# nktoan/h-edit

Measured on AMD Instinct MI355X. Metric: edited images/sec (512^2, 50 steps, K Langevin), higher is better.
Workload: dtype bf16

## Files before the change

h-edit_amd/csrc/attn.hip:

```cpp
#include "common.h"
#include "kernels.h"
#include <type_traits>

namespace {

typedef __attribute__((ext_vector_type(4))) unsigned u32x4;

__device__ __forceinline__ float fast_exp2(float x) { return __builtin_amdgcn_exp2f(x); }
#ifndef SA_BURST
#define SA_BURST 0
#endif

template <int D>
struct HeadCfg {
  static constexpr int DP = (D + 15) / 16 * 16;
  static constexpr int DK = DP / 16;
  static constexpr int DT = (D + 31) / 32;
  static constexpr int KS = DP + 8;
  static constexpr int DCH = D / 8;
};

__device__ __forceinline__ bf16x8 pack_p8(const float* p) {
  union { uint32_t u[4]; bf16x8 v; } x;
  x.u[0] = pack_bf16x2(p[0], p[1]);
// ... 427 lines not shown
      block(integral_constant<int, 0>{}, false_type{}, false_type{}, U);
      block(integral_constant<int, 1>{}, false_type{}, false_type{}, U + 1);
      if (QG == 2) hand_over((U >> 2) + 1); else hand_over((U >> 1) + 2);
      block(integral_constant<int, 2>{}, false_type{}, false_type{}, U + 2);
      block(integral_constant<int, 3>{}, false_type{}, false_type{}, U + 3);
      U = 4;
    }
    for (; U + 6 <= TU; U += 4) {
      if (QG == 1) hand_over((U >> 1) + 1);
      block(integral_constant<int, 0>{}, false_type{}, pin, U);
      block(integral_constant<int, 1>{}, false_type{}, pin, U + 1);
      if (QG == 2) hand_over((U >> 2) + 1); else hand_over((U >> 1) + 2);
      block(integral_constant<int, 2>{}, false_type{}, pin, U + 2);
      block(integral_constant<int, 3>{}, false_type{}, pin, U + 3);
    }
    {
      if (QG == 1) hand_over((U >> 1) + 1);
      block(integral_constant<int, 0>{}, true_type{}, pin, U);
      block(integral_constant<int, 1>{}, true_type{}, pin, U + 1);
      if (U + 2 < TU) {
        if (QG == 2) hand_over((U >> 2) + 1); else hand_over((U >> 1) + 2);
        block(integral_constant<int, 2>{}, true_type{}, pin, U + 2);
        block(integral_constant<int, 3>{}, true_type{}, pin, U + 3);
      }
    }
    {
      bf16x8 (&pf_last)[2] = pfb;
      constexpr int AL = NS - 1;
      if constexpr (PV16) {
#pragma unroll
        for (int gq = 0; gq < 2; ++gq)
#pragma unroll
          for (int dt = 0; dt < DT16; ++dt)
            o16[AL][gq][dt] = MFMA_16x16x32_ST(vf16[dt], pf_last[gq], o16[AL][gq][dt], 0, 0, 0);
      } else {
#pragma unroll
      for (int dt = 0; dt < DT; ++dt) o[AL][dt] = MFMA_32x32x16_ST(vf[dt][0], pf_last[0], o[AL][dt], 0, 0, 0);
#pragma unroll
      for (int dt = 0; dt < DT; ++dt) o[AL][dt] = MFMA_32x32x16_ST(vf[dt][1], pf_last[1], o[AL][dt], 0, 0, 0);
      }
    }
  };

  constexpr int dl = D - (DT - 1) * 32;
  constexpr int r1 = (dl & 3) + 4 * (dl >> 3);
  constexpr int h1 = (dl >> 2) & 1;
  auto denom16 = [&](int a, int gq) __attribute__((always_inline)) {
    return __shfl(o16[a][gq][D / 16][D % 4], 16 * ((D % 16) / 4) + (lane & 15), 64);
  };
  auto denom = [&](int a) __attribute__((always_inline)) {
    if (ONES) return __shfl(o[a][DT - 1][ONES ? r1 : 0], ql + 32 * h1, 64);
    return l_run[a] + __shfl_xor(l_run[a], 32, 64);
  };
  auto write_out = [&](const f32x16 (&acc)[DT], float inv, int q_row) __attribute__((always_inline)) {
    if (q_row < p.N) {
      bf16_t* op = p.out + ((long)b * p.N + q_row) * p.ldo + h * D;
#pragma unroll
      for (int dt = 0; dt < DT; ++dt)
#pragma unroll
        for (int gg = 0; gg < 4; ++gg) {
          const int d0 = dt * 32 + 8 * gg + 4 * hi;
          if (d0 < D) {
            uint2 w;
            w.x = pack_bf16x2(acc[dt][gg * 4 + 0] * inv, acc[dt][gg * 4 + 1] * inv);
            w.y = pack_bf16x2(acc[dt][gg * 4 + 2] * inv, acc[dt][gg * 4 + 3] * inv);
            *reinterpret_cast<uint2*>(op + d0) = w;
          }
        }
    }
  };
  {
    constexpr bool CAN_PIN = D != 64;
    int redo = 1;
    if (CAN_PIN && TU >= 6 && !(p.test_flags & 2)) {
      pass(true_type{});
      bool bad = false;
#pragma unroll
      for (int a = 0; a < NS; ++a) {
        constexpr float DEN_MAX = HEDIT_F16 ? 0x1p15f : 0x1p60f;
        if constexpr (PV16) bad |= !(denom16(a, 0) < DEN_MAX) || !(denom16(a, 1) < DEN_MAX);
        else bad |= !(denom(a) < DEN_MAX);
      }
      redo = __syncthreads_or(bad ? 1 : 0);
    }
    if (redo) pass(false_type{});
  }
  if constexpr (PV16) {
#pragma unroll
    for (int g = 0; g < 2; ++g)
#pragma unroll
      for (int gq = 0; gq < 2; ++gq) {
        const float inv = 1.0f / denom16(g, gq);
        const int q_row = qblk * (128 * QG) + wave * (32 * QG) + g * 32 + gq * 16 + (lane & 15);
        if (q_row < p.N) {
          bf16_t* op = p.out + ((long)b * p.N + q_row) * p.ldo + h * D;
#pragma unroll
          for (int dt = 0; dt < DT16; ++dt) {
            const int d0 = dt * 16 + 4 * (lane >> 4);
            if (d0 < D) {
              uint2 w;
              w.x = pack_bf16x2(o16[g][gq][dt][0] * inv, o16[g][gq][dt][1] * inv);
              w.y = pack_bf16x2(o16[g][gq][dt][2] * inv, o16[g][gq][dt][3] * inv);
              *reinterpret_cast<uint2*>(op + d0) = w;
            }
          }
        }
      }
  } else if (QG == 2) {
#pragma unroll
    for (int g = 0; g < 2; ++g) write_out(o[g], 1.0f / denom(g), q_base + g * 32);
  } else {
    if (NS == 2) {
      const float m = fmaxf(m_run[0], m_run[NS - 1]);
      const float f0 = fast_exp2(m_run[0] - m), f1 = fast_exp2(m_run[NS - 1] - m);
      if (!ONES) l_run[0] = l_run[0] * f0 + l_run[NS - 1] * f1;
#pragma unroll
      for (int dt = 0; dt < DT; ++dt)
#pragma unroll
        for (int r = 0; r < 16; ++r) o[0][dt][r] = o[0][dt][r] * f0 + o[NS - 1][dt][r] * f1;
    }
    write_out(o[0], 1.0f / denom(0), q_base);
  }
}

template <int D, int QG, int NS>
int launch_self(const SelfAttnParams& p, hipStream_t st) {
  using C = SelfCfg<D, QG>;
#ifdef SA_OCC1
  constexpr int LDS = C::TOTAL > 84 * 1024 ? C::TOTAL : 84 * 1024;
#else
  constexpr int LDS = C::TOTAL;
#endif
  if (int rc = hedit_dyn_lds(reinterpret_cast<const void*>(&self_attn_kernel<D, QG, NS>), LDS)) return rc;
  dim3 grid(cdiv(p.N, 128 * QG) * p.heads * p.B);
  hipLaunchKernelGGL((self_attn_kernel<D, QG, NS>), grid, dim3(256), LDS, st, p);
  LAUNCH_CHECK();
  return HEDIT_OK;
}

constexpr int CTXP = HEDIT_CTXP;
constexpr int WS = 100;

template <int D>
struct CrossSmem {
  using H = HeadCfg<D>;
  static constexpr int K_BYTES = 96 * H::KS * 2;
  static constexpr int V_BYTES = H::DT * 32 * WS * 2;
  static constexpr int MIX_BYTES = 96 * WS * 2;
  static constexpr int BV_BYTES = 96 * 4;
  static constexpr int TOTAL = K_BYTES + V_BYTES + MIX_BYTES + BV_BYTES;
};

template <int D>
__global__ __launch_bounds__(256, (D <= 80 ? 2 : 1)) void cross_attn_kernel(CrossAttnParams p) {
  using H = HeadCfg<D>;
  using S = CrossSmem<D>;
  extern __shared__ __attribute__((aligned(16))) char smem[];
  bf16_t* sK = reinterpret_cast<bf16_t*>(smem);
  bf16_t* sV = reinterpret_cast<bf16_t*>(smem + S::K_BYTES);
  bf16_t* sM = reinterpret_cast<bf16_t*>(smem + S::K_BYTES + S::V_BYTES);
  float* sB = reinterpret_cast<float*>(smem + S::K_BYTES + S::V_BYTES + S::MIX_BYTES);

  const int tid = threadIdx.x, lane = tid & 63, wave = tid >> 6;
  const int ql = lane & 31, hi = lane >> 5;
  const int h = blockIdx.y;
  const int item = blockIdx.z;
  const bool is_pair = item < p.n_pairs;
  const int b0 = is_pair ? p.pair_src[item] : p.singles[item - p.n_pairs];
  const int b1 = is_pair ? p.pair_tar[item] : -1;
  const int q_row = blockIdx.x * 128 + wave * 32 + ql;
  const bool q_ok = q_row < p.N;

  for (int i = tid; i < (S::K_BYTES + S::V_BYTES) / 8; i += 256) reinterpret_cast<uint2*>(smem)[i] = make_uint2(0, 0);
  if (is_pair) {
    const bf16_t* src = p.mixT + (long)item * 96 * 96;
    for (int i = tid; i < 96 * 12; i += 256) {
      const int row = i / 12, c = i - row * 12;
      const uint4 u = *reinterpret_cast<const uint4*>(src + row * 96 + c * 8);
      uint2* dst = reinterpret_cast<uint2*>(sM + row * WS + c * 8);
      dst[0] = make_uint2(u.x, u.y);
      dst[1] = make_uint2(u.z, u.w);
    }
    if (tid < 96) sB[tid] = p.bvec[(long)item * 96 + tid];
  }
  __syncthreads();

  auto stage = [&](int b) {
    const bf16_t* kbase = p.k + (long)b * CTXP * p.ldk + h * D;
    for (int idx = tid; idx < CTXP * H::DCH; idx += 256) {
      const int row = idx / H::DCH, c = idx - row * H::DCH;
      *reinterpret_cast<uint4*>(sK + row * H::KS + c * 8) =
          *reinterpret_cast<const uint4*>(kbase + (long)row * p.ldk + c * 8);
    }
    const bf16_t* vbase = p.vt + (long)h * D * p.ldvt + (long)b * CTXP;
    for (int idx = tid; idx < D * (CTXP / 8); idx += 256) {
      const int row = idx / (CTXP / 8), c = idx - row * (CTXP / 8);
      const uint4 u = *reinterpret_cast<const uint4*>(vbase + (long)row * p.ldvt + c * 8);
      uint2* dst = reinterpret_cast<uint2*>(sV + row * WS + c * 8);
      dst[0] = make_uint2(u.x, u.y);
      dst[1] = make_uint2(u.z, u.w);
    }
  };

  auto load_q = [&](int b, bf16x8* qf) {
    const bf16_t* qp = p.q + ((long)b * p.N + (q_ok ? q_row : 0)) * p.ldq + h * D;
#pragma unroll
    for (int ks = 0; ks < H::DK; ++ks) {
      const int c = ks * 16 + hi * 8;
      union { uint4 u; bf16x8 v; } x;
      x.u = make_uint4(0, 0, 0, 0);
      if (q_ok && c < D) x.u = *reinterpret_cast<const uint4*>(qp + c);
      qf[ks] = x.v;
    }
  };

  auto probs = [&](const bf16x8* qf, float (*pr)[16]) {
    float mx = -1e30f;
#pragma unroll
    for (int nt = 0; nt < 3; ++nt) {
      f32x16 s;
#pragma unroll
      for (int r = 0; r < 16; ++r) s[r] = 0.f;
#pragma unroll
      for (int ks = 0; ks < H::DK; ++ks) {
        const bf16x8 kf = *reinterpret_cast<const bf16x8*>(sK + (nt * 32 + ql) * H::KS + ks * 16 + hi * 8);
        s = MFMA_32x32x16_ST(kf, qf[ks], s, 0, 0, 0);
      }
#pragma unroll
      for (int r = 0; r < 16; ++r) {
        const int n = nt * 32 + (r & 3) + 8 * (r >> 2) + 4 * hi;
        const float v = n < HEDIT_MAXW ? s[r] : -1e30f;
        pr[nt][r] = v;
        mx = fmaxf(mx, v);
      }
    }
    mx = fmaxf(mx, __shfl_xor(mx, 32, 64));
    float ls = 0.f;
#pragma unroll
    for (int nt = 0; nt < 3; ++nt)
#pragma unroll
      for (int r = 0; r < 16; ++r) { pr[nt][r] = fast_exp2(pr[nt][r] - mx); ls += pr[nt][r]; }
    ls += __shfl_xor(ls, 32, 64);
    const float inv = 1.0f / ls;
#pragma unroll
    for (int nt = 0; nt < 3; ++nt)
#pragma unroll
      for (int r = 0; r < 16; ++r) pr[nt][r] *= inv;
  };

  auto accumulate_store = [&](int which, float (*pr)[16]) {
    if (p.store == nullptr || !q_ok) return;
    float* dst = p.store + ((((long)item * 2 + which) * p.heads + h) * p.N + q_row) * HEDIT_MAXW;
#pragma unroll
    for (int nt = 0; nt < 3; ++nt)
#pragma unroll
      for (int r = 0; r < 16; ++r) {
        const int n = nt * 32 + (r & 3) + 8 * (r >> 2) + 4 * hi;
        if (n < HEDIT_MAXW) dst[n] += pr[nt][r];
      }
  };

  auto pv_and_write = [&](int b, const bf16x8 (*pf)[2]) {
    f32x16 o[H::DT];
#pragma unroll
    for (int dt = 0; dt < H::DT; ++dt) {
#pragma unroll
      for (int r = 0; r < 16; ++r) o[dt][r] = 0.f;
#pragma unroll
      for (int nt = 0; nt < 3; ++nt)
#pragma unroll
        for (int s2 = 0; s2 < 2; ++s2) {
          const bf16x8 vf = read_perm_frag(sV, dt * 32 + ql, WS, nt * 32 + 16 * s2 + 4 * hi);
          o[dt] = MFMA_32x32x16_ST(vf, pf[nt][s2], o[dt], 0, 0, 0);
        }
    }
    if (q_ok) {
      bf16_t* op = p.out + ((long)b * p.N + q_row) * p.ldo + h * D;
#pragma unroll
      for (int dt = 0; dt < H::DT; ++dt)
#pragma unroll
        for (int g = 0; g < 4; ++g) {
          const int d0 = dt * 32 + 8 * g + 4 * hi;
          if (d0 < D) {
            uint2 w;
            w.x = pack_bf16x2(o[dt][g * 4 + 0], o[dt][g * 4 + 1]);
            w.y = pack_bf16x2(o[dt][g * 4 + 2], o[dt][g * 4 + 3]);
            *reinterpret_cast<uint2*>(op + d0) = w;
          }
        }
    }
  };

  bf16x8 qf[H::DK];
  float pr[3][16];
  bf16x8 pf[3][2];

  stage(b0);
  __syncthreads();
  load_q(b0, qf);
  probs(qf, pr);
  if (is_pair) accumulate_store(0, pr);
#pragma unroll
  for (int nt = 0; nt < 3; ++nt) { pf[nt][0] = pack_p8(pr[nt]); pf[nt][1] = pack_p8(pr[nt] + 8); }
  pv_and_write(b0, pf);
  if (!is_pair) return;

  f32x16 mix[3];
#pragma unroll
  for (int nt = 0; nt < 3; ++nt) {
#pragma unroll
    for (int r = 0; r < 16; ++r) mix[nt][r] = 0.f;
#pragma unroll
    for (int wt = 0; wt < 3; ++wt)
#pragma unroll
      for (int s2 = 0; s2 < 2; ++s2) {
        const bf16x8 mf = read_perm_frag(sM, nt * 32 + ql, WS, wt * 32 + 16 * s2 + 4 * hi);
        mix[nt] = MFMA_32x32x16_ST(mf, pf[wt][s2], mix[nt], 0, 0, 0);
      }
  }
  __syncthreads();
  stage(b1);
  __syncthreads();
  load_q(b1, qf);
  probs(qf, pr);
#pragma unroll
  for (int nt = 0; nt < 3; ++nt)
#pragma unroll
    for (int g = 0; g < 4; ++g) {
      const f32x4 bv = *reinterpret_cast<const f32x4*>(sB + nt * 32 + 8 * g + 4 * hi);
#pragma unroll
      for (int j = 0; j < 4; ++j) pr[nt][g * 4 + j] = mix[nt][g * 4 + j] + bv[j] * pr[nt][g * 4 + j];
    }
  accumulate_store(1, pr);
#pragma unroll
  for (int nt = 0; nt < 3; ++nt) { pf[nt][0] = pack_p8(pr[nt]); pf[nt][1] = pack_p8(pr[nt] + 8); }
  pv_and_write(b1, pf);
}

template <int D>
int launch_cross(const CrossAttnParams& p, hipStream_t st) {
  using S = CrossSmem<D>;
  if (int rc = hedit_dyn_lds(reinterpret_cast<const void*>(&cross_attn_kernel<D>), S::TOTAL)) return rc;
  dim3 grid(cdiv(p.N, 128), p.heads, p.n_pairs + p.n_single);
  hipLaunchKernelGGL((cross_attn_kernel<D>), grid, dim3(256), S::TOTAL, st, p);
  LAUNCH_CHECK();
  return HEDIT_OK;
}

template <bool STORE>
__global__ __launch_bounds__(256) void attn_probs_kernel(AttnProbsParams p) {
  __shared__ float qs[16][168];
  extern __shared__ float sc_rows[];
  const int bh = blockIdx.y, h = bh % p.heads;
  int b = bh / p.heads;
  if constexpr (STORE) {
    const int pair = b >> 1;
    b = (b & 1) ? p.pair_tar[pair] : p.pair_src[pair];
  }
  const int bq = (STORE && p.qk_src) ? p.qk_src[b] : b;
  const int q0 = blockIdx.x * 16, tid = threadIdx.x;
  for (int i = tid; i < 16 * p.d; i += 256) {
    const int r = i / p.d, c = i % p.d;
    const int q = q0 + r;
    qs[r][c] = q < p.N ? bf16_to_f32(p.q[((long)bq * p.N + q) * p.ldq + h * p.d + c]) : 0.f;
  }
  __syncthreads();
  float* out = STORE ? sc_rows : p.probs + ((long)bh * p.N + q0) * p.M;
  const int rows = min(16, p.N - q0);
  for (int m = tid; m < p.M; m += 256) {
    const bf16_t* kp = p.k + ((long)bq * p.kstride + m) * p.ldk + h * p.d;
    float acc[16];
#pragma unroll
    for (int r = 0; r < 16; ++r) acc[r] = 0.f;
    for (int c = 0; c < p.d; c += 8) {
      const uint4 raw = *reinterpret_cast<const uint4*>(kp + c);
      const uint32_t w[4] = {raw.x, raw.y, raw.z, raw.w};
#pragma unroll
      for (int j = 0; j < 8; ++j) {
        const float kv = (j & 1) ? st_hi(w[j >> 1]) : st_lo(w[j >> 1]);
#pragma unroll
        for (int r = 0; r < 16; ++r) acc[r] += qs[r][c + j] * kv;
      }
    }
    for (int r = 0; r < rows; ++r) out[(long)r * p.M + m] = acc[r];
  }
  __syncthreads();
  const int wave = tid >> 6, lane = tid & 63;
  for (int r = wave; r < rows; r += 4) {
    float* row = out + (long)r * p.M;
    float mx = -3.0e38f;
    for (int m = lane; m < p.M; m += 64) mx = fmaxf(mx, row[m]);
#pragma unroll
    for (int o = 32; o > 0; o >>= 1) mx = fmaxf(mx, __shfl_xor(mx, o, 64));
    float sum = 0.f;
    for (int m = lane; m < p.M; m += 64) {
      const float e = exp2f(row[m] - mx);
      row[m] = e;
      sum += e;
    }
#pragma unroll
    for (int o = 32; o > 0; o >>= 1) sum += __shfl_xor(sum, o, 64);
    const float inv = 1.0f / sum;
    if constexpr (STORE) {
      float* acc_row = p.probs + ((long)bh * p.N + q0 + r) * p.M;
      for (int m = lane; m < p.M; m += 64) acc_row[m] += row[m] * inv;
    } else {
      for (int m = lane; m < p.M; m += 64) row[m] *= inv;
    }
  }
}

__global__ __launch_bounds__(256) void attn_apply_kernel(AttnProbsParams p) {
  constexpr int CH = 64;
  __shared__ float ps[16][CH + 1];
  __shared__ float vs[160][CH + 1];
  const int bh = blockIdx.y, b = bh / p.heads, h = bh % p.heads;
  const int q0 = blockIdx.x * 16, tid = threadIdx.x;
  const int rows = min(16, p.N - q0), d = p.d;
  const int nout = 16 * d;
  float acc[10];
#pragma unroll
  for (int i = 0; i < 10; ++i) acc[i] = 0.f;
  const float* pin = p.probs + ((long)bh * p.N + q0) * p.M;
  for (int m0 = 0; m0 < p.M; m0 += CH) {
    const int mc = min(CH, p.M - m0);
    for (int i = tid; i < 16 * CH; i += 256) {
      const int r = i / CH, c = i % CH;
      ps[r][c] = (r < rows && c < mc) ? pin[(long)r * p.M + m0 + c] : 0.f;
    }
    for (int i = tid; i < d * CH; i += 256) {
      const int r = i / CH, c = i % CH;
      vs[r][c] = c < mc ? bf16_to_f32(p.vt[(long)(h * d + r) * p.ldvt + (long)b * p.kstride + m0 + c]) : 0.f;
    }
    __syncthreads();
#pragma unroll
    for (int i = 0; i < 10; ++i) {
      const int o = tid + i * 256;
      if (o < nout) {
        const int r = o / d, c = o % d;
        float a = acc[i];
        for (int m = 0; m < CH; ++m) a += ps[r][m] * vs[c][m];
        acc[i] = a;
      }
    }
    __syncthreads();
  }
#pragma unroll
  for (int i = 0; i < 10; ++i) {
    const int o = tid + i * 256;
    if (o < nout) {
      const int r = o / d, c = o % d;
      if (r < rows) p.out[((long)b * p.N + q0 + r) * p.ldo + h * d + c] = f32_to_bf16(acc[i]);
    }
  }
}

}

int attn_probs_launch(const AttnProbsParams& p, hipStream_t st) {
  ARG_CHECK(p.d % 8 == 0 && p.d <= 160, "attn_probs: head dim must be a multiple of 8, at most 160");
  ARG_CHECK(p.ldq % 8 == 0 && p.ldk % 8 == 0, "attn_probs: strides");
  ARG_CHECK(p.M > 0 && p.N > 0 && p.M <= p.kstride, "attn_probs: extents");
  hipLaunchKernelGGL(attn_probs_kernel<false>, dim3(cdiv(p.N, 16), p.B * p.heads), dim3(256), 0, st, p);
  LAUNCH_CHECK();
  return HEDIT_OK;
}

int attn_self_store_launch(const AttnProbsParams& p, hipStream_t st) {
  ARG_CHECK(p.d % 8 == 0 && p.d <= 160 && p.ldq % 8 == 0 && p.ldk % 8 == 0, "attn_self_store: head dim / strides");
  ARG_CHECK(p.M > 0 && p.N > 0 && p.M <= 1024 && p.M <= p.kstride && p.pair_src && p.pair_tar && p.probs, "attn_self_store: extents");
  const int lds = 16 * p.M * (int)sizeof(float);
  if (int rc = hedit_dyn_lds(reinterpret_cast<const void*>(&attn_probs_kernel<true>), lds)) return rc;
  hipLaunchKernelGGL(attn_probs_kernel<true>, dim3(cdiv(p.N, 16), 2 * p.B * p.heads), dim3(256), lds, st, p);
  LAUNCH_CHECK();
  return HEDIT_OK;
}

int attn_apply_launch(const AttnProbsParams& p, hipStream_t st) {
  ARG_CHECK(p.d % 8 == 0 && p.d <= 160, "attn_apply: head dim must be a multiple of 8, at most 160");
  ARG_CHECK(p.M > 0 && p.N > 0 && p.M <= p.kstride, "attn_apply: extents");
  hipLaunchKernelGGL(attn_apply_kernel, dim3(cdiv(p.N, 16), p.B * p.heads), dim3(256), 0, st, p);
  LAUNCH_CHECK();
  return HEDIT_OK;
}

int self_attn_launch(const SelfAttnParams& p_in, hipStream_t st) {
  SelfAttnParams p = p_in;
  p.test_flags = hedit_test_flags();
  ARG_CHECK(p.N % 64 == 0, "self_attn: N must be a multiple of 64");
  ARG_CHECK(p.ldq % 8 == 0 && p.ldk % 8 == 0 && p.ldvt % 8 == 0 && p.ldo % 4 == 0, "self_attn: strides");
  switch (p.d) {
    case 32: return launch_self<32, 2, 2>(p, st);
    case 40: return launch_self<40, 2, 2>(p, st);
    case 64: return launch_self<64, 2, 2>(p, st);
    case 80: return launch_self<80, 1, 1>(p, st);
    case 160: return launch_self<160, 1, 1>(p, st);
    default:
// ... 20 lines not shown
```

h-edit_amd/csrc/c_api.hip:

```cpp
#include "../../include/hedit.h"
#include <exception>
#include <map>
#include <mutex>
#include <new>
#include <set>
#include <utility>

#include "common.h"
#include "kernels.h"

static thread_local std::string g_last_error;
void hedit_set_error(const std::string& msg) { g_last_error = msg; }

int hedit_abi_catch() noexcept {
  try {
    try {
      throw;
    } catch (const std::bad_alloc&) {
      g_last_error = "out of host memory inside libhedit_hip";
    } catch (const std::exception& e) {
      g_last_error = std::string("C++ exception inside libhedit_hip: ") + e.what();
    } catch (...) {
      g_last_error = "unknown C++ exception inside libhedit_hip";
    }
// ... 133 lines not shown
int hedit_k_gemm_plan_splits(int M, int N, int K, int chunk_kt) { return gemm_plan_splits(M, N, K, chunk_kt); }

int hedit_k_gemm(const void* A, const void* W, const float* bias, const void* residual, void* C, int M, int N,
                 int K, int lda, int ldc, int ldr, int mode, int Hin, int Win, int Cin, int Hout, int Wout,
                 int splits, void* partial_ws, void* stream) try {
  ARG_CHECK(A && W && C, "gemm args");
  GemmParams p{};
  p.A = reinterpret_cast<const bf16_t*>(A);
  p.W = reinterpret_cast<const bf16_t*>(W);
  p.M = M; p.N = N; p.K = K; p.lda = lda; p.mode = mode;
  p.Hin = Hin; p.Win = Win; p.Cin = Cin; p.Hout = Hout; p.Wout = Wout;
  p.bias = bias;
  p.residual = reinterpret_cast<const bf16_t*>(residual);
  p.ldr = ldr;
  p.C = reinterpret_cast<bf16_t*>(C);
  p.ldc = ldc;
  if (splits < 0) {
    const int kt = K / 64;
    const int s = gemm_pick_splits(M, N, K, -splits);
    p.chunk_kt = (kt + s - 1) / s;
    return gemm_launch(p, 1, nullptr, S(stream));
  }
  const int s = gemm_pick_splits(M, N, K, splits);
  return gemm_launch(p, s, reinterpret_cast<float*>(partial_ws), S(stream));
} catch (...) { return hedit_abi_catch(); }

int hedit_k_conv_gn(const void* A, const void* W, const float* bias, const void* residual, void* C, int M, int N, int K, int ldc,
                    int ldr, int mode, int Hin, int Win, int Cin, int Hout, int Wout, int splits, void* partial_ws, float* gn_part,
                    void* stream) try {
  ARG_CHECK(A && W && C && gn_part, "conv_gn args");
  GemmParams p{};
  p.A = reinterpret_cast<const bf16_t*>(A);
  p.W = reinterpret_cast<const bf16_t*>(W);
  p.M = M; p.N = N; p.K = K; p.lda = Cin; p.mode = mode;
  p.Hin = Hin; p.Win = Win; p.Cin = Cin; p.Hout = Hout; p.Wout = Wout;
  p.bias = bias;
  p.residual = reinterpret_cast<const bf16_t*>(residual);
  p.ldr = ldr;
  p.C = reinterpret_cast<bf16_t*>(C);
  p.ldc = ldc;
  p.gn_part = gn_part;
  if (splits < 0) {
    const int kt = K / 64;
    const int s = gemm_pick_splits(M, N, K, -splits);
    p.chunk_kt = (kt + s - 1) / s;
    return gemm_launch(p, 1, nullptr, S(stream));
  }
  const int s = gemm_pick_splits(M, N, K, splits);
  return gemm_launch(p, s, reinterpret_cast<float*>(partial_ws), S(stream));
} catch (...) { return hedit_abi_catch(); }

int hedit_k_groupnorm_from_parts(const void* x, void* y, const float* gamma, const float* beta, int B, int HW, int C, int G,
                                 float eps, int silu, const float* part_a, int ca, const float* part_b, int cb, void* ws,
                                 void* stream) try {
  ARG_CHECK(x && y && gamma && beta && part_a && ws, "groupnorm_from_parts args");
  return groupnorm_from_parts_launch(reinterpret_cast<const bf16_t*>(x), reinterpret_cast<bf16_t*>(y), gamma, beta, B, HW, C, G,
                                     eps, silu, part_a, ca, part_b, cb, reinterpret_cast<float*>(ws), S(stream));
} catch (...) { return hedit_abi_catch(); }

int hedit_k_pack_geglu(const float* w, const float* bias, void* w_packed_bf16, float* bias_packed, int inner, int K,
                       void* stream) try {
  ARG_CHECK(w && w_packed_bf16, "pack_geglu args");
  int rc = pack_geglu_rows_launch(w, reinterpret_cast<bf16_t*>(w_packed_bf16), nullptr, 2 * inner, K, S(stream));
  if (rc != HEDIT_OK || !bias) return rc;
  ARG_CHECK(bias_packed, "pack_geglu: bias_packed");
  return pack_geglu_rows_launch(bias, nullptr, bias_packed, 2 * inner, 1, S(stream));
} catch (...) { return hedit_abi_catch(); }

int hedit_k_gemm_geglu(const void* A, const void* w_packed, const float* bias_packed, void* C, int M, int inner, int K,
                       int lda, int ldc, void* stream) try {
  ARG_CHECK(A && w_packed && C, "gemm_geglu args");
  GemmParams p{};
  p.A = reinterpret_cast<const bf16_t*>(A);
  p.W = reinterpret_cast<const bf16_t*>(w_packed);
  p.M = M; p.N = 2 * inner; p.K = K; p.lda = lda; p.mode = 0;
  p.bias = bias_packed;
  p.C = reinterpret_cast<bf16_t*>(C);
  p.ldc = ldc;
  p.geglu = 1;
  return gemm_launch(p, 1, nullptr, S(stream));
} catch (...) { return hedit_abi_catch(); }

int hedit_k_ffn_channels(void) { return ffn_fused_channels(); }
size_t hedit_k_ffn_stream_bytes(int with_outer_layers) { return ffn_stream_bytes(with_outer_layers, with_outer_layers); }
size_t hedit_k_ffn_bias_bytes(void) { return ffn_bias_bytes(); }

int hedit_k_ffn_pack(const float* w1, const float* b1, const float* w2, const float* w_pre, const float* w_post, void* stream_out,
                     float* bias1_out, void* stream) try {
  ARG_CHECK(w1 && b1 && w2 && stream_out && bias1_out && ((w_pre == nullptr) == (w_post == nullptr)), "ffn_pack args");
  const int outer = w_pre != nullptr;
  bf16_t* so = reinterpret_cast<bf16_t*>(stream_out);
  int rc = ffn_pack_launch(w1, 1, outer, outer, so, S(stream));
  if (rc == HEDIT_OK) rc = ffn_pack_launch(w2, 2, outer, outer, so, S(stream));
  if (rc == HEDIT_OK && outer) rc = ffn_pack_launch(w_pre, 0, 1, 1, so, S(stream));
  if (rc == HEDIT_OK && outer) rc = ffn_pack_launch(w_post, 3, 1, 1, so, S(stream));
  if (rc != HEDIT_OK) return rc;
  return ffn_pack_bias_launch(b1, bias1_out, S(stream));
} catch (...) { return hedit_abi_catch(); }

int hedit_k_ffn_fused(const void* x, int64_t ldx, const float* gamma, const float* beta, float eps, const void* w_stream,
                      const float* bias1_packed, const float* bias2, void* out, int64_t ldo, int M, int C, void* stream) try {
  FfnParams f{};
  f.x = reinterpret_cast<const bf16_t*>(x); f.ldx = (long)ldx; f.gamma = gamma; f.beta = beta; f.eps = eps;
  f.stream = reinterpret_cast<const bf16_t*>(w_stream); f.bias1p = bias1_packed; f.bias2 = bias2;
  f.out = reinterpret_cast<bf16_t*>(out); f.ldo = (long)ldo; f.M = M; f.C = C;
  return ffn_fused_launch(f, S(stream));
} catch (...) { return hedit_abi_catch(); }

int hedit_k_ffn_chain(const void* a, int64_t lda, const void* t1, int64_t ldt1, const void* x, int64_t ldx, const float* bias_pre,
                      const float* gamma, const float* beta, float eps, const void* w_stream, const float* bias1_packed, const float* bias2,
                      const float* bias_post, void* out, int64_t ldo, int M, int C, void* stream) try {
  ARG_CHECK(a && t1 && x, "ffn_chain args");
  FfnParams f{};
  f.a = reinterpret_cast<const bf16_t*>(a); f.lda = (long)lda;
  f.x = reinterpret_cast<const bf16_t*>(t1); f.ldx = (long)ldt1;
  f.r2 = reinterpret_cast<const bf16_t*>(x); f.ldr2 = (long)ldx;
  f.bias_pre = bias_pre; f.bias_post = bias_post;
  f.gamma = gamma; f.beta = beta; f.eps = eps;
  f.stream = reinterpret_cast<const bf16_t*>(w_stream); f.bias1p = bias1_packed; f.bias2 = bias2;
  f.out = reinterpret_cast<bf16_t*>(out); f.ldo = (long)ldo; f.M = M; f.C = C;
  return ffn_fused_launch(f, S(stream));
} catch (...) { return hedit_abi_catch(); }

size_t hedit_k_lin_chain_stream_bytes(int n_out) { return lin_chain_stream_bytes(n_out == 3 ? 4 : 2); }

int hedit_k_lin_chain_pack(const float* w_pre, const float* w0, const float* w1, const float* w2, float scale0, void* stream_out,
                           void* stream) try {
  ARG_CHECK(w_pre && w0 && stream_out && ((w1 == nullptr) == (w2 == nullptr)), "lin_chain_pack args");
  const int layers = w1 ? 4 : 2;
  bf16_t* so = reinterpret_cast<bf16_t*>(stream_out);
  int rc = lin_chain_pack_launch(w_pre, 0, 1.f, layers, so, S(stream));
  if (rc == HEDIT_OK) rc = lin_chain_pack_launch(w0, 1, scale0, layers, so, S(stream));
  if (rc == HEDIT_OK && w1) rc = lin_chain_pack_launch(w1, 2, 1.f, layers, so, S(stream));
  if (rc == HEDIT_OK && w1) rc = lin_chain_pack_launch(w2, 3, 1.f, layers, so, S(stream));
  return rc;
} catch (...) { return hedit_abi_catch(); }

int hedit_k_lin_chain(const void* a, int64_t lda, const void* r1, int64_t ldr1, const float* gn_ss, int rows_per_image,
                      const float* bias_pre, const float* gamma, const float* beta, float eps, const void* w_stream, void* out_mid,
                      int64_t ldmid, void* out_q, int64_t ldq, void* out_k, int64_t ldk, void* out, int64_t ldo, int M, int C,
                      void* stream) try {
  LinChainParams c{};
  c.a = reinterpret_cast<const bf16_t*>(a); c.lda = (long)lda; c.r1 = reinterpret_cast<const bf16_t*>(r1); c.ldr1 = (long)ldr1;
  c.bias_pre = bias_pre; c.gamma = gamma; c.beta = beta; c.eps = eps; c.stream = reinterpret_cast<const bf16_t*>(w_stream);
  c.out_mid = reinterpret_cast<bf16_t*>(out_mid); c.ldmid = (long)ldmid; c.out = reinterpret_cast<bf16_t*>(out); c.ldo = (long)ldo;
  c.M = M; c.C = C; c.gn_ss = gn_ss; c.rows_per_image = rows_per_image;
  c.out_q = reinterpret_cast<bf16_t*>(out_q); c.ldq = (long)ldq; c.out_k = reinterpret_cast<bf16_t*>(out_k); c.ldk = (long)ldk;
  return lin_chain_launch(c, S(stream));
} catch (...) { return hedit_abi_catch(); }

int hedit_storage_is_f16(void) { return HEDIT_F16; }

int hedit_test_set_flags(int flags) try {
  ARG_CHECK(flags >= 0 && flags <= 31, "hedit_test_set_flags: bit 0 drained ring waits, bit 1 exact self-attention pass, bit 2 pixel-UNet GroupNorm statistics path flipped, bit 3 no persistent linear kernel, bit 4 narrow one-launch GroupNorm");
  g_test_flags.store(flags, std::memory_order_relaxed);
  return HEDIT_OK;
} catch (...) { return hedit_abi_catch(); }

int hedit_k_lin_chain_sched(const void* a, int64_t lda, const void* r1, int64_t ldr1, const float* gn_ss, int rows_per_image,
                            const float* bias_pre, const float* gamma, const float* beta, float eps, const void* w_stream, void* out_mid,
                            int64_t ldmid, void* out_q, int64_t ldq, void* out_k, int64_t ldk, void* out, int64_t ldo, int M, int C,
                            int sched, void* stream) try {
  LinChainParams c{};
  c.a = reinterpret_cast<const bf16_t*>(a); c.lda = (long)lda; c.r1 = reinterpret_cast<const bf16_t*>(r1); c.ldr1 = (long)ldr1;
  c.bias_pre = bias_pre; c.gamma = gamma; c.beta = beta; c.eps = eps; c.stream = reinterpret_cast<const bf16_t*>(w_stream);
  c.out_mid = reinterpret_cast<bf16_t*>(out_mid); c.ldmid = (long)ldmid; c.out = reinterpret_cast<bf16_t*>(out); c.ldo = (long)ldo;
  c.M = M; c.C = C; c.gn_ss = gn_ss; c.rows_per_image = rows_per_image;
  c.out_q = reinterpret_cast<bf16_t*>(out_q); c.ldq = (long)ldq; c.out_k = reinterpret_cast<bf16_t*>(out_k); c.ldk = (long)ldk;
  return lin_chain_launch_sched(c, sched, S(stream));
} catch (...) { return hedit_abi_catch(); }

size_t hedit_k_groupnorm_ws_bytes(int B, int HW, int C) { return groupnorm_ws_bytes(B, HW, C); }

int hedit_k_groupnorm_affine(const void* x, const float* gamma, const float* beta, int B, int HW, int C, int G, float eps, void* ws,
                             float* ss_out, void* stream) try {
  ARG_CHECK(x && gamma && beta && ws && ss_out, "groupnorm_affine args");
  const float* ss = nullptr;
  int rc = groupnorm_affine_launch(reinterpret_cast<const bf16_t*>(x), gamma, beta, B, HW, C, G, eps, reinterpret_cast<float*>(ws), S(stream), &ss);
  if (rc != HEDIT_OK) return rc;
  HIP_TRY(hipMemcpyAsync(ss_out, ss, (size_t)B * C * 2 * sizeof(float), hipMemcpyDeviceToDevice, S(stream)));
  return HEDIT_OK;
} catch (...) { return hedit_abi_catch(); }

int hedit_k_groupnorm(const void* x, void* y, const float* gamma, const float* beta, int B, int HW, int C, int G,
                      float eps, int silu, void* ws, void* stream) try {
  ARG_CHECK(x && y && gamma && beta && ws, "groupnorm args");
  return groupnorm_launch(reinterpret_cast<const bf16_t*>(x), reinterpret_cast<bf16_t*>(y), gamma, beta, B, HW, C, G,
                          eps, silu, reinterpret_cast<float*>(ws), S(stream));
} catch (...) { return hedit_abi_catch(); }

int hedit_k_layernorm(const void* x, void* y, const float* gamma, const float* beta, int64_t rows, int C, float eps,
                      void* stream) try {
  ARG_CHECK(x && y && gamma && beta, "layernorm args");
  return layernorm_launch(reinterpret_cast<const bf16_t*>(x), reinterpret_cast<bf16_t*>(y), gamma, beta, (long)rows, C, eps, S(stream));
} catch (...) { return hedit_abi_catch(); }

int hedit_k_geglu(const void* x, void* y, int64_t rows, int inner, void* stream) try {
  ARG_CHECK(x && y, "geglu args");
  return geglu_launch(reinterpret_cast<const bf16_t*>(x), reinterpret_cast<bf16_t*>(y), (long)rows, inner, S(stream));
} catch (...) { return hedit_abi_catch(); }

int hedit_k_self_attn(const void* q, int ldq, const void* k, int ldk, const void* vt, int64_t ldvt, void* out, int ldo,
                      int B, int N, int heads, int d, const int32_t* qk_src, const int32_t* kv_src, void* stream) try {
  ARG_CHECK(q && k && vt && out, "self_attn args");
  SelfAttnParams p{};
  p.q = reinterpret_cast<const bf16_t*>(q); p.ldq = ldq;
  p.k = reinterpret_cast<const bf16_t*>(k); p.ldk = ldk;
  p.vt = reinterpret_cast<const bf16_t*>(vt); p.ldvt = (long)ldvt;
  p.out = reinterpret_cast<bf16_t*>(out); p.ldo = ldo;
  p.B = B; p.N = N; p.heads = heads; p.d = d; p.qk_src = qk_src; p.kv_src = kv_src;
  return self_attn_launch(p, S(stream));
} catch (...) { return hedit_abi_catch(); }

int hedit_k_cross_attn(const void* q, int ldq, const void* k, int ldk, const void* vt, int64_t ldvt, void* out, int ldo,
                       int B, int N, int heads, int d, const hedit_p2p_plan* plan, float* store, void* stream) try {
  ARG_CHECK(q && k && vt && out && plan, "cross_attn args");
  CrossAttnParams p{};
  p.q = reinterpret_cast<const bf16_t*>(q); p.ldq = ldq;
  p.k = reinterpret_cast<const bf16_t*>(k); p.ldk = ldk;
  p.vt = reinterpret_cast<const bf16_t*>(vt); p.ldvt = (long)ldvt;
  p.out = reinterpret_cast<bf16_t*>(out); p.ldo = ldo;
  p.B = B; p.N = N; p.heads = heads; p.d = d;
  p.n_pairs = plan->n_pairs; p.pair_src = plan->pair_src; p.pair_tar = plan->pair_tar;
  p.mixT = reinterpret_cast<const bf16_t*>(plan->mixT); p.bvec = plan->bvec;
  p.singles = plan->singles; p.n_single = plan->n_single;
  p.store = store;
  return cross_attn_launch(p, S(stream));
} catch (...) { return hedit_abi_catch(); }

int hedit_k_attn_probs(const void* q, int ldq, const void* k, int ldk, float* probs, int B, int N, int M, int kstride,
                       int heads, int d, void* stream) try {
  ARG_CHECK(q && k && probs, "attn_probs args");
  AttnProbsParams p{};
  p.q = reinterpret_cast<const bf16_t*>(q); p.ldq = ldq;
  p.k = reinterpret_cast<const bf16_t*>(k); p.ldk = ldk;
  p.probs = probs; p.B = B; p.N = N; p.M = M; p.kstride = kstride; p.heads = heads; p.d = d;
  return attn_probs_launch(p, S(stream));
} catch (...) { return hedit_abi_catch(); }

int hedit_k_attn_apply(const float* probs, const void* vt, int64_t ldvt, void* out, int ldo, int B, int N, int M,
                       int kstride, int heads, int d, void* stream) try {
  ARG_CHECK(probs && vt && out, "attn_apply args");
  AttnProbsParams p{};
  p.probs = const_cast<float*>(probs);
  p.vt = reinterpret_cast<const bf16_t*>(vt); p.ldvt = (long)ldvt;
  p.out = reinterpret_cast<bf16_t*>(out); p.ldo = ldo;
  p.B = B; p.N = N; p.M = M; p.kstride = kstride; p.heads = heads; p.d = d;
  return attn_apply_launch(p, S(stream));
} catch (...) { return hedit_abi_catch(); }

int hedit_k_pack_conv3x3(const float* w, void* out, int O, int I, void* stream) try {
  ARG_CHECK(w && out, "pack args");
  return pack_conv3x3_launch(w, reinterpret_cast<bf16_t*>(out), O, I, S(stream));
} catch (...) { return hedit_abi_catch(); }

int hedit_k_f32_to_bf16(const float* x, void* y, int64_t n, void* stream) try {
  ARG_CHECK(x && y, "cast args");
  return f32_to_bf16_launch(x, reinterpret_cast<bf16_t*>(y), (long)n, S(stream));
} catch (...) { return hedit_abi_catch(); }

int hedit_k_groupnorm_stats(const void* x, void* y, const float* gamma, const float* beta, int B, int HW, int C, int G,
                            float eps, int silu, void* ws, float* stats, void* stream) try {
  ARG_CHECK(x && y && gamma && beta && ws && stats, "groupnorm_stats args");
  return groupnorm_launch(reinterpret_cast<const bf16_t*>(x), reinterpret_cast<bf16_t*>(y), gamma, beta, B, HW, C, G,
                          eps, silu, reinterpret_cast<float*>(ws), S(stream), stats);
} catch (...) { return hedit_abi_catch(); }

size_t hedit_k_groupnorm_bwd_ws_bytes(int B, int HW, int C) { return groupnorm_bwd_ws_bytes(B, HW, C); }

int hedit_k_groupnorm_bwd(const void* x, const void* dy, const void* add, void* dx, const float* gamma, const float* beta,
                          const float* stats, int B, int HW, int C, int G, int silu, void* ws, void* stream) try {
  ARG_CHECK(x && dy && dx && gamma && beta && stats && ws, "groupnorm_bwd args");
  return groupnorm_bwd_launch(reinterpret_cast<const bf16_t*>(x), reinterpret_cast<const bf16_t*>(dy),
                              reinterpret_cast<const bf16_t*>(add), reinterpret_cast<bf16_t*>(dx), gamma, beta, stats, B, HW, C,
                              G, silu, reinterpret_cast<float*>(ws), S(stream));
} catch (...) { return hedit_abi_catch(); }

int hedit_k_softmax_rows(const float* s, void* p, int64_t rows, int N, float scale, void* stream) try {
  ARG_CHECK(s && p, "softmax_rows args");
  return softmax_rows_launch(s, reinterpret_cast<bf16_t*>(p), (long)rows, N, scale, S(stream));
} catch (...) { return hedit_abi_catch(); }

int hedit_k_softmax_blockdiag(const float* s, void* p, int64_t rows, int T, int ld, float scale, void* stream) try {
  ARG_CHECK(s && p, "softmax_blockdiag args");
  return softmax_blockdiag_launch(s, reinterpret_cast<bf16_t*>(p), (long)rows, T, ld, scale, S(stream));
} catch (...) { return hedit_abi_catch(); }

int hedit_k_softmax_bwd(const void* p, const float* dp, void* ds, int64_t rows, int N, float scale, void* stream) try {
  ARG_CHECK(p && dp && ds, "softmax_bwd args");
  return softmax_bwd_launch(reinterpret_cast<const bf16_t*>(p), dp, reinterpret_cast<bf16_t*>(ds), (long)rows, N, scale, S(stream));
} catch (...) { return hedit_abi_catch(); }

int hedit_k_transpose(const void* src, void* dst, int R, int C, void* stream) try {
  ARG_CHECK(src && dst, "transpose args");
  return transpose_bf16_launch(reinterpret_cast<const bf16_t*>(src), reinterpret_cast<bf16_t*>(dst), R, C, S(stream));
} catch (...) { return hedit_abi_catch(); }

int hedit_k_sum2x2(const void* du, void* dx, int B, int H, int W, int C, void* stream) try {
  ARG_CHECK(du && dx, "sum2x2 args");
  return sum2x2_launch(reinterpret_cast<const bf16_t*>(du), reinterpret_cast<bf16_t*>(dx), B, H, W, C, S(stream));
} catch (...) { return hedit_abi_catch(); }

int hedit_k_pack_conv3x3_dgrad(const float* w, void* out, int O, int I, void* stream) try {
  ARG_CHECK(w && out, "pack args");
  return pack_conv3x3_dgrad_launch(w, reinterpret_cast<bf16_t*>(out), O, I, S(stream));
} catch (...) { return hedit_abi_catch(); }

// ... 110 lines not shown
```

Measured before the change: 2.612.

## Walk several query tiles per cross-attention block, reusing staged K/V

The cross-attention kernel now processes a run of consecutive 128-row query tiles per block, staging the context K/V (and the pair mix matrix) into LDS once and reusing it across tiles. The next tile's Q fragments are prefetched while the current tile computes. For pairs it keeps both source and target K/V resident when LDS allows, and it skips the padded third-subtile MFMAs and exponentials. The run length is chosen from CU count to keep enough blocks in flight. This trades fewer blocks and some parallelism for less redundant global-to-LDS staging, and a test flag keeps the old one-tile path.

Measured after the change: 2.627 (median of 6 runs). Within noise of the previous version (+0.6%).

```diff
diff --git a/h-edit_amd/csrc/attn.hip b/h-edit_amd/csrc/attn.hip
--- a/h-edit_amd/csrc/attn.hip
+++ b/h-edit_amd/csrc/attn.hip
@@ -603,7 +603,7 @@
 };
 
 template <int D>
-__global__ __launch_bounds__(256, (D <= 80 ? 2 : 1)) void cross_attn_kernel(CrossAttnParams p) {
+__global__ __launch_bounds__(256, (D <= 80 ? 2 : 1)) void cross_attn_tile_kernel(CrossAttnParams p) {
   using H = HeadCfg<D>;
   using S = CrossSmem<D>;
   extern __shared__ __attribute__((aligned(16))) char smem[];
@@ -789,11 +789,322 @@
 }
 
 template <int D>
+struct CrossWalk {
+  using S = CrossSmem<D>;
+  static constexpr int ROW_BYTES = S::K_BYTES + S::V_BYTES;
+  static constexpr int PAIR_BYTES = S::MIX_BYTES + S::BV_BYTES;
+  static constexpr int BLOCKS_PAIR = D <= 80 ? 2 : 1, BLOCKS_PLAIN = D <= 80 ? 4 : 2;
+  static constexpr bool BOTH = BLOCKS_PAIR * (2 * ROW_BYTES + PAIR_BYTES) <= 160 * 1024;
+  static constexpr int TOTAL_PAIR = (BOTH ? 2 : 1) * ROW_BYTES + PAIR_BYTES;
+  static_assert(BLOCKS_PAIR * TOTAL_PAIR <= 160 * 1024 && BLOCKS_PLAIN * ROW_BYTES <= 160 * 1024, "LDS of the declared blocks per CU");
+};
+
+template <int D, bool PAIRS>
+__global__ __launch_bounds__(256, (PAIRS ? CrossWalk<D>::BLOCKS_PAIR : CrossWalk<D>::BLOCKS_PLAIN)) void cross_attn_kernel(CrossAttnParams p, int run) {
+  using H = HeadCfg<D>;
+  using S = CrossSmem<D>;
+  using W = CrossWalk<D>;
+  extern __shared__ __attribute__((aligned(16))) char smem[];
+  char* row0 = smem;
+  char* row1 = smem + (W::BOTH ? W::ROW_BYTES : 0);
+  bf16_t* sM = reinterpret_cast<bf16_t*>(smem + (W::BOTH ? 2 : 1) * W::ROW_BYTES);
+  float* sB = reinterpret_cast<float*>(smem + (W::BOTH ? 2 : 1) * W::ROW_BYTES + S::MIX_BYTES);
+  auto kof = [](char* row) { return reinterpret_cast<bf16_t*>(row); };
+  auto vof = [](char* row) { return reinterpret_cast<bf16_t*>(row + S::K_BYTES); };
+
+  const int tid = threadIdx.x, lane = tid & 63, wave = tid >> 6;
+  const int ql = lane & 31, hi = lane >> 5;
+  const int h = blockIdx.y;
+  const int item = blockIdx.z;
+  const bool is_pair = PAIRS && item < p.n_pairs;
+  const int b0 = is_pair ? p.pair_src[item] : p.singles[item - p.n_pairs];
+  const int b1 = is_pair ? p.pair_tar[item] : -1;
+  const int t_begin = blockIdx.x * run;
+  const int t_end = min(t_begin + run, (p.N + 127) / 128);
+  int q_row = t_begin * 128 + wave * 32 + ql;
+  bool q_ok = q_row < p.N;
+
+  auto load_q = [&](int b, int t, bf16x8* qf) {
+    const int row = t * 128 + wave * 32 + ql;
+    const bool ok = row < p.N;
+    const bf16_t* qp = p.q + ((long)b * p.N + (ok ? row : 0)) * p.ldq + h * D;
+#pragma unroll
+    for (int ks = 0; ks < H::DK; ++ks) {
+      const int c = ks * 16 + hi * 8;
+      union { uint4 u; bf16x8 v; } x;
+      x.u = *reinterpret_cast<const uint4*>(qp + (c < D ? c : 0));
+      if (!(ok && c < D)) x.u = make_uint4(0, 0, 0, 0);
+      qf[ks] = x.v;
+    }
+  };
+
+  auto zero_pad = [&](char* row) {
+    bf16_t* sK = kof(row);
+    bf16_t* sV = vof(row);
+    if (H::DP > D)
+      for (int r = tid; r < CTXP; r += 256) *reinterpret_cast<uint4*>(sK + r * H::KS + D) = make_uint4(0, 0, 0, 0);
+    for (int i = tid; i < (96 - CTXP) * (H::DP / 8); i += 256) {
+      const int r = CTXP + i / (H::DP / 8), c = i % (H::DP / 8);
+      *reinterpret_cast<uint4*>(sK + r * H::KS + c * 8) = make_uint4(0, 0, 0, 0);
+    }
+    for (int i = tid; i < (H::DT * 32 - D) * (CTXP / 4); i += 256) {
+      const int r = D + i / (CTXP / 4), c = i % (CTXP / 4);
+      *reinterpret_cast<uint2*>(sV + r * WS + c * 4) = make_uint2(0, 0);
+    }
+  };
+
+  auto stage = [&](int b, char* dst_row) {
+    bf16_t* sK = kof(dst_row);
+    bf16_t* sV = vof(dst_row);
+    constexpr int KN = CTXP * H::DCH, KI = (KN + 255) / 256;
+    constexpr int VN = D * (CTXP / 8), VI = (VN + 255) / 256;
+    uint4 kr[KI], vr[VI];
+    const bf16_t* kbase = p.k + (long)b * CTXP * p.ldk + h * D;
+#pragma unroll
+    for (int i = 0; i < KI; ++i) {
+      const int idx = min(tid + i * 256, KN - 1);
+      const int row = idx / H::DCH, c = idx - row * H::DCH;
+      kr[i] = *reinterpret_cast<const uint4*>(kbase + (long)row * p.ldk + c * 8);
+    }
+    const bf16_t* vbase = p.vt + (long)h * D * p.ldvt + (long)b * CTXP;
+#pragma unroll
+    for (int i = 0; i < VI; ++i) {
+      const int idx = min(tid + i * 256, VN - 1);
+      const int row = idx / (CTXP / 8), c = idx - row * (CTXP / 8);
+      vr[i] = *reinterpret_cast<const uint4*>(vbase + (long)row * p.ldvt + c * 8);
+    }
+#pragma unroll
+    for (int i = 0; i < KI; ++i) {
+      const int idx = tid + i * 256;
+      const int row = idx / H::DCH, c = idx - row * H::DCH;
+      if (idx < KN) *reinterpret_cast<uint4*>(sK + row * H::KS + c * 8) = kr[i];
+    }
+#pragma unroll
+    for (int i = 0; i < VI; ++i) {
+      const int idx = tid + i * 256;
+      const int row = idx / (CTXP / 8), c = idx - row * (CTXP / 8);
+      if (idx < VN) {
+        uint2* dst = reinterpret_cast<uint2*>(sV + row * WS + c * 8);
+        dst[0] = make_uint2(vr[i].x, vr[i].y);
+        dst[1] = make_uint2(vr[i].z, vr[i].w);
+      }
+    }
+  };
+
+  auto probs = [&](const bf16_t* sK, const bf16x8* qf, float (*pr)[16]) {
+    float mx = -1e30f;
+#pragma unroll
+    for (int nt = 0; nt < 3; ++nt) {
+      f32x16 s;
+#pragma unroll
+      for (int r = 0; r < 16; ++r) s[r] = 0.f;
+#pragma unroll
+      for (int ks = 0; ks < H::DK; ++ks) {
+        const bf16x8 kf = *reinterpret_cast<const bf16x8*>(sK + (nt * 32 + ql) * H::KS + ks * 16 + hi * 8);
+        s = MFMA_32x32x16_ST(kf, qf[ks], s, 0, 0, 0);
+      }
+#pragma unroll
+      for (int r = 0; r < (nt == 2 ? 8 : 16); ++r) {
+        const int n = nt * 32 + (r & 3) + 8 * (r >> 2) + 4 * hi;
+        const float v = n < HEDIT_MAXW ? s[r] : -1e30f;
+        pr[nt][r] = v;
+        mx = fmaxf(mx, v);
+      }
+    }
+    mx = fmaxf(mx, __shfl_xor(mx, 32, 64));
+    float ls = 0.f;
+#pragma unroll
+    for (int nt = 0; nt < 3; ++nt)
+#pragma unroll
+      for (int r = 0; r < (nt == 2 ? 8 : 16); ++r) { pr[nt][r] = fast_exp2(pr[nt][r] - mx); ls += pr[nt][r]; }
+    ls += __shfl_xor(ls, 32, 64);
+    const float inv = 1.0f / ls;
+#pragma unroll
+    for (int nt = 0; nt < 3; ++nt)
+#pragma unroll
+      for (int r = 0; r < (nt == 2 ? 8 : 16); ++r) pr[nt][r] *= inv;
+  };
+
+  auto accumulate_store = [&](int which, float (*pr)[16]) {
+    if (p.store == nullptr || !q_ok) return;
+    float* dst = p.store + ((((long)item * 2 + which) * p.heads + h) * p.N + q_row) * HEDIT_MAXW;
+#pragma unroll
+    for (int nt = 0; nt < 3; ++nt)
+#pragma unroll
+      for (int r = 0; r < (nt == 2 ? 8 : 16); ++r) {
+        const int n = nt * 32 + (r & 3) + 8 * (r >> 2) + 4 * hi;
+        if (n < HEDIT_MAXW) dst[n] += pr[nt][r];
+      }
+  };
+
+  auto pack = [&](float (*pr)[16], bf16x8 (*pf)[2]) {
+#pragma unroll
+    for (int nt = 0; nt < 3; ++nt) {
+      pf[nt][0] = pack_p8(pr[nt]);
+      if (nt < 2) pf[nt][1] = pack_p8(pr[nt] + 8);
+    }
+  };
+
+  auto pv_and_write = [&](const bf16_t* sV, int b, const bf16x8 (*pf)[2]) {
+    f32x16 o[H::DT];
+#pragma unroll
+    for (int dt = 0; dt < H::DT; ++dt) {
+#pragma unroll
+      for (int r = 0; r < 16; ++r) o[dt][r] = 0.f;
+#pragma unroll
+      for (int nt = 0; nt < 3; ++nt)
+#pragma unroll
+        for (int s2 = 0; s2 < (nt == 2 ? 1 : 2); ++s2) {
+          const bf16x8 vf = read_perm_frag(sV, dt * 32 + ql, WS, nt * 32 + 16 * s2 + 4 * hi);
+          o[dt] = MFMA_32x32x16_ST(vf, pf[nt][s2], o[dt], 0, 0, 0);
+        }
+    }
+    if (q_ok) {
+      bf16_t* op = p.out + ((long)b * p.N + q_row) * p.ldo + h * D;
+#pragma unroll
+      for (int dt = 0; dt < H::DT; ++dt)
+#pragma unroll
+        for (int g = 0; g < 4; ++g) {
+          const int d0 = dt * 32 + 8 * g + 4 * hi;
+          if (d0 < D) {
+            uint2 w;
+            w.x = pack_bf16x2(o[dt][g * 4 + 0], o[dt][g * 4 + 1]);
+            w.y = pack_bf16x2(o[dt][g * 4 + 2], o[dt][g * 4 + 3]);
+            *reinterpret_cast<uint2*>(op + d0) = w;
+          }
+        }
+    }
+  };
+
+  bf16x8 qc[2][H::DK], qn[2][H::DK];
+  float pr[3][16];
+  bf16x8 pf[3][2];
+
+  load_q(b0, t_begin, qc[0]);
+  if (is_pair) load_q(b1, t_begin, qc[1]);
+  zero_pad(row0);
+  stage(b0, row0);
+  if (is_pair) {
+    const bf16_t* src = p.mixT + (long)item * 96 * 96;
+    constexpr int MN = 96 * 12, MI = (MN + 255) / 256;
+    uint4 mr[MI];
+#pragma unroll
+    for (int i = 0; i < MI; ++i) mr[i] = *reinterpret_cast<const uint4*>(src + min(tid + i * 256, MN - 1) * 8);
+#pragma unroll
+    for (int i = 0; i < MI; ++i) {
+      const int idx = tid + i * 256;
+      const int row = idx / 12, c = idx - row * 12;
+      if (idx < MN) {
+        uint2* dst = reinterpret_cast<uint2*>(sM + row * WS + c * 8);
+        dst[0] = make_uint2(mr[i].x, mr[i].y);
+        dst[1] = make_uint2(mr[i].z, mr[i].w);
+      }
+    }
+    if (tid < 96) sB[tid] = p.bvec[(long)item * 96 + tid];
+    if (W::BOTH) {
+      zero_pad(row1);
+      stage(b1, row1);
+    }
+  }
+  __syncthreads();
+
+  for (int t = t_begin; t < t_end; ++t) {
+    const bool more = t + 1 < t_end;
+    if (more) {
+      load_q(b0, t + 1, qn[0]);
+      if (is_pair) load_q(b1, t + 1, qn[1]);
+    }
+    q_row = t * 128 + wave * 32 + ql;
+    q_ok = q_row < p.N;
+    __atomic_signal_fence(__ATOMIC_SEQ_CST);
+
+    probs(kof(row0), qc[0], pr);
+    if (is_pair) accumulate_store(0, pr);
+    pack(pr, pf);
+    pv_and_write(vof(row0), b0, pf);
+
+    if (is_pair) {
+      f32x16 mix[3];
+#pragma unroll
+      for (int nt = 0; nt < 3; ++nt) {
+#pragma unroll
+        for (int r = 0; r < 16; ++r) mix[nt][r] = 0.f;
+#pragma unroll
+        for (int wt = 0; wt < 3; ++wt)
+#pragma unroll
+          for (int s2 = 0; s2 < (wt == 2 ? 1 : 2); ++s2) {
+            const bf16x8 mf = read_perm_frag(sM, nt * 32 + ql, WS, wt * 32 + 16 * s2 + 4 * hi);
+            mix[nt] = MFMA_32x32x16_ST(mf, pf[wt][s2], mix[nt], 0, 0, 0);
+          }
+      }
+      if (!W::BOTH) {
+        __syncthreads();
+        stage(b1, row1);
+        __syncthreads();
+      }
+      probs(kof(row1), qc[1], pr);
+#pragma unroll
+      for (int nt = 0; nt < 3; ++nt)
+#pragma unroll
+        for (int g = 0; g < (nt == 2 ? 2 : 4); ++g) {
+          const f32x4 bv = *reinterpret_cast<const f32x4*>(sB + nt * 32 + 8 * g + 4 * hi);
+#pragma unroll
+          for (int j = 0; j < 4; ++j) pr[nt][g * 4 + j] = mix[nt][g * 4 + j] + bv[j] * pr[nt][g * 4 + j];
+        }
+      accumulate_store(1, pr);
+      pack(pr, pf);
+      pv_and_write(vof(row1), b1, pf);
+      if (!W::BOTH && more) {
+        __syncthreads();
+        stage(b0, row0);
+        __syncthreads();
+      }
+    }
+
+    if (more) {
+#pragma unroll
+      for (int ks = 0; ks < H::DK; ++ks) {
+        qc[0][ks] = qn[0][ks];
+        if (is_pair) qc[1][ks] = qn[1][ks];
+      }
+    }
+  }
+}
+
+inline int cross_run(int tiles, int units_per_tile, int slots) {
+  for (int r = 4; r > 1; --r) {
+    const int nruns = cdiv(tiles, r);
+    if ((long)nruns * units_per_tile >= slots) return cdiv(tiles, nruns);
+  }
+  return 1;
+}
+
+template <int D>
 int launch_cross(const CrossAttnParams& p, hipStream_t st) {
   using S = CrossSmem<D>;
-  if (int rc = hedit_dyn_lds(reinterpret_cast<const void*>(&cross_attn_kernel<D>), S::TOTAL)) return rc;
-  dim3 grid(cdiv(p.N, 128), p.heads, p.n_pairs + p.n_single);
-  hipLaunchKernelGGL((cross_attn_kernel<D>), grid, dim3(256), S::TOTAL, st, p);
+  using W = CrossWalk<D>;
+  const int items = p.n_pairs + p.n_single, tiles = cdiv(p.N, 128);
+  const int flags = hedit_test_flags();
+  if (flags & 32) {
+    if (int rc = hedit_dyn_lds(reinterpret_cast<const void*>(&cross_attn_tile_kernel<D>), S::TOTAL)) return rc;
+    dim3 grid(tiles, p.heads, items);
+    hipLaunchKernelGGL((cross_attn_tile_kernel<D>), grid, dim3(256), S::TOTAL, st, p);
+    LAUNCH_CHECK();
+    return HEDIT_OK;
+  }
+  int cus = 0;
+  if (int rc = hedit_cu_count(&cus)) return rc;
+  const bool pairs = p.n_pairs > 0;
+  int run = cross_run(tiles, p.heads * items, cus * (pairs ? W::BLOCKS_PAIR : W::BLOCKS_PLAIN));
+  if ((flags >> 8) & 15) run = std::min(tiles, (flags >> 8) & 15);
+  dim3 grid(cdiv(tiles, run), p.heads, items);
+  if (pairs) {
+    if (int rc = hedit_dyn_lds(reinterpret_cast<const void*>(&cross_attn_kernel<D, true>), W::TOTAL_PAIR)) return rc;
+    hipLaunchKernelGGL((cross_attn_kernel<D, true>), grid, dim3(256), W::TOTAL_PAIR, st, p, run);
+  } else {
+    if (int rc = hedit_dyn_lds(reinterpret_cast<const void*>(&cross_attn_kernel<D, false>), W::ROW_BYTES)) return rc;
+    hipLaunchKernelGGL((cross_attn_kernel<D, false>), grid, dim3(256), W::ROW_BYTES, st, p, run);
+  }
   LAUNCH_CHECK();
   return HEDIT_OK;
 }
diff --git a/h-edit_amd/csrc/c_api.hip b/h-edit_amd/csrc/c_api.hip
--- a/h-edit_amd/csrc/c_api.hip
+++ b/h-edit_amd/csrc/c_api.hip
@@ -309,7 +309,7 @@
 int hedit_storage_is_f16(void) { return HEDIT_F16; }
 
 int hedit_test_set_flags(int flags) try {
-  ARG_CHECK(flags >= 0 && flags <= 31, "hedit_test_set_flags: bit 0 drained ring waits, bit 1 exact self-attention pass, bit 2 pixel-UNet GroupNorm statistics path flipped, bit 3 no persistent linear kernel, bit 4 narrow one-launch GroupNorm");
+  ARG_CHECK(flags >= 0 && (flags & ~0xF3F) == 0, "hedit_test_set_flags: bit 0 drained ring waits, bit 1 exact self-attention pass, bit 2 pixel-UNet GroupNorm statistics path flipped, bit 3 no persistent linear kernel, bit 4 narrow one-launch GroupNorm, bit 5 one-tile cross-attention, bits 8-11 forced cross-attention run length");
   g_test_flags.store(flags, std::memory_order_relaxed);
   return HEDIT_OK;
 } catch (...) { return hedit_abi_catch(); }
```
